# vlongle/pixie

Measured on AMD Instinct MI355X. Metric: voxels/s (128^3 U-Net fwd) + MPM particle-steps/s, higher is better.
Workload: dtype f32 (operands split fp16 hi+lo, 3 f16 MFMAs/product, fp32 accumulate); 1 GPU; 128^3x64 feature grid -> SegmentationUNet+RegressionUNet forward (+argmax/one-hot combine), 1 scene per GPU per step; grid=128, feature_channels=64, parallelism=scene-parallel x1, executor=c+hip_graph

## Files before the change

pixie_amd/csrc/conv16_body.h:

```cpp
#pragma once
#include <type_traits>

#include "conv16_device.h"

namespace pixie {

template <int KS, int MB, int NB, bool EX = false, bool SP = false, int SK = 0, bool PAIR = false>
__device__ __forceinline__ void conv3d_f16x3_body(const Conv16Args& A) {
    static_assert(!PAIR || (MB == 2 && !EX && !SP && SK == 0), "pair form: the plain f16x3 body with 64 c_out per quartet");
    static_assert(!SP || (KS == 3 && NB == 4 && !EX), "sub-pixel path: 3^3, two x parities x two voxel blocks per wave");
    static_assert(SK == 0 || (!EX && !SP), "folded skip (SK: 1 register-fed, 2 staged through LDS): f16x3, no sub-pixel form");
    extern __shared__ uint4 smem16[];
    constexpr int PAD = (KS == 3) ? 1 : 0;
    constexpr int NW = 4, NT = 64 * NW;
    const int bufsz = 4 * A.CS;

    const int tid = threadIdx.x;
    const int lane = tid & 63;
    const int quartet = PAIR ? __builtin_amdgcn_readfirstlane(tid >> 8) : 0;
    const int wave = PAIR ? (tid >> 6) & 3 : tid >> 6;
    const int qtid = PAIR ? tid & 255 : tid;
    const int kh = lane >> 5;
    const int l31 = lane & 31;

    int t = blockIdx.x;
    {
        const int per = (A.n_tiles + 7) >> 3;
        const int cand = (t & 7) * per + (t >> 3);
        if ((A.n_tiles & 7) == 0) t = cand;
    }
    int par = 0;
    if constexpr (SP) { par = t & 3; t >>= 2; }
    const int py = par & 1, pz = par >> 1;
    const int tx = t % A.tiles_x; t /= A.tiles_x;
    const int ty = t % A.tiles_y;
    const int tz = t / A.tiles_y;
    const int ox0 = tx * A.TX, oy0 = ty * A.TY, oz0 = tz * A.TZ;
    const int cout0 = (PAIR ? 2 * (int)blockIdx.y + quartet : (int)blockIdx.y) * (MB * 32);
    const int lx0 = SP ? ox0 - 1 : ox0 * A.stride - PAD;
    const int ly0 = SP ? oy0 - 1 + py : oy0 * A.stride - PAD;
    const int lz0 = SP ? oz0 - 1 + pz : oz0 * A.stride - PAD;
// ... 31 lines not shown
    }

    float bound = A.in_bound;
    if (A.amax0) {
        bound = __uint_as_float(*A.amax0);
        if (A.amax1) bound = fmaxf(bound, __uint_as_float(*A.amax1));
    }
    const int ex = EX ? 0 : scale_exponent(bound);
    const float sx = pow2i(ex);

    f32x16 acc[MB][NB];
#pragma unroll
    for (int mb = 0; mb < MB; ++mb)
#pragma unroll
        for (int nb = 0; nb < NB; ++nb)
#pragma unroll
            for (int r = 0; r < 16; ++r) acc[mb][nb][r] = 0.0f;

    const int KG = A.cin >> 3;
    const size_t tap_stride = (size_t)KG * A.coutp;
    const size_t plane = (size_t)(SP ? 64 : KS * KS * KS) * tap_stride;
    const uint4* wHi = A.w16 + kW16HeaderU4 + (size_t)kh * A.coutp + cout0 + l31 + (size_t)(par * 16) * tap_stride;
    const uint4* wLo = wHi + plane;
    const float* wF = A.wf + (size_t)kh * A.coutp + cout0 + l31;

    constexpr int TAPS = KS * KS * KS;
#include "conv16_stage.h"
#include "conv16_taps.h"

    float inv2 = 0.0f;
    {
        const int c_begin = A.partial ? (int)blockIdx.z * A.chunks_per_slice * 16 : 0;
        const int c_end = A.partial ? min(A.cin, c_begin + A.chunks_per_slice * 16) : A.cin;
        if constexpr (PAIR) {
            const int n_chunks = (c_end - c_begin) >> 4;
            const int half = (A.CS + 1) >> 1;
            const int s0 = quartet ? half : 0, s1 = quartet ? A.CS : half;
#pragma unroll 1
            for (int h = -1; h < 2 * n_chunks; ++h) {
                const int k = h >> 1;
                const bool stage = (h < 0 || ((h + quartet) & 1) == 0) && k + 1 < n_chunks;
                const bool multiply = h >= 0 && ((h + quartet) & 1) != 0;
                if (stage) stage_chunk(c_begin + 16 * (k + 1), smem16 + ((k + 1) & 1) * bufsz, qtid, NT, s0, s1);
                if (multiply) mfma_chunk(c_begin + 16 * k, smem16 + (k & 1) * bufsz);
                if (h & 1) __syncthreads();
            }
        } else {
            for (int c_base = c_begin; c_base < c_end; c_base += 16) {
                __syncthreads();
                stage_chunk(c_base, smem16, tid, NT, 0, A.CS);
                __syncthreads();
                mfma_chunk(c_base, smem16);
            }
        }
#include "conv16_skip.h"
    }

#include "conv16_epilogue.h"
}

template <int KS, int MB, int NB>
__global__ __launch_bounds__(256, 2) void conv3d_f16x3_kernel(Conv16Args A) {
    conv3d_f16x3_body<KS, MB, NB>(A);
}
template <int KS, int NB>
__global__ __launch_bounds__(512, 1) void conv3d_f16x3_pair_kernel(Conv16Args A) {
    conv3d_f16x3_body<KS, 2, NB, false, false, 0, true>(A);
}
template <int KS, int MB, int NB, bool STAGED>
__global__ __launch_bounds__(256, 2) void conv3d_f16x3_skip_kernel(Conv16Args A) {
    conv3d_f16x3_body<KS, MB, NB, false, false, STAGED ? 2 : 1>(A);
}
template <int KS, int MB, int NB>
__global__ __launch_bounds__(256, 2) void conv3d_exact_kernel(Conv16Args A) {
    conv3d_f16x3_body<KS, MB, NB, true>(A);
}
template <int MB>
__global__ __launch_bounds__(256, 2) void conv3d_f16x3_subpixel_kernel(Conv16Args A) {
    conv3d_f16x3_body<3, MB, 4, false, true>(A);
}
__global__ __launch_bounds__(256, 2) void conv3d_f16x3_c64_fullres_kernel(Conv16Args A) {
    conv3d_f16x3_body<3, 2, 4>(A);
}

}
```

pixie_amd/csrc/conv3d_f16x3.hip:

```cpp
#include <hip/hip_runtime.h>

#include <cstdlib>

#include "../../include/pixie_hip.h"
#include "common.h"
#include "conv_plan.h"
#include "conv_launch.h"
#include "conv16_device.h"
#include "conv16_body.h"
#include "conv_stat_kernels.h"
#include "conv_pack_kernels.h"

namespace pixie {

bool conv_exact_v1() { return getenv("PIXIE_CONV_EXACT_V1") != nullptr; }

ConvShape conv_shape_of(const pixie_conv_desc* d) {
    ConvShape s;
    s.c0 = d->c0; s.c1 = d->c1; s.c_out = d->c_out;
    s.in_d = d->in_d; s.in_h = d->in_h; s.in_w = d->in_w;
    s.ksize = d->ksize; s.stride = d->stride; s.upsample = d->upsample;
    s.out_d = d->out_d; s.out_h = d->out_h; s.out_w = d->out_w;
    s.skip_c0 = d->skip_c0; s.skip_c1 = d->skip_c1;
    s.w16 = d->d_w16 != nullptr; s.subpixel = d->w16_subpixel != 0; s.workspace = d->d_workspace != nullptr; s.skip = d->d_skip_w16 != nullptr;
    s.exact_v1 = conv_exact_v1();
    return s;
}

using ConvKernel = void (*)(Conv16Args);
static ConvKernel conv16_kernel(const ConvPlan& p, bool skip = false, int skip_c0 = 0) {
    if (p.path == CONV_F16X3_SUBPIXEL) return p.MB == 2 ? conv3d_f16x3_subpixel_kernel<2> : conv3d_f16x3_subpixel_kernel<1>;
    if (p.fullres) return conv3d_f16x3_c64_fullres_kernel;
#define PX_CONV16_PICK(KS_, MB_, NB_)                                                                \
    if (p.KS == KS_ && p.MB == MB_ && p.NB == NB_)                                                   \
        return p.path == CONV_EXACT_TILED ? conv3d_exact_kernel<KS_, MB_, NB_>                       \
                                          : (!skip ? conv3d_f16x3_kernel<KS_, MB_, NB_>                                \
                                                   : ((skip_c0 & 8) ? conv3d_f16x3_skip_kernel<KS_, MB_, NB_, true> : conv3d_f16x3_skip_kernel<KS_, MB_, NB_, false>));
    PX_CONV_VARIANTS(PX_CONV16_PICK)
#undef PX_CONV16_PICK
    return nullptr;
}

#ifdef PIXIE_DIAG
static int g_conv_keep_four_wave = 0;
#endif
static size_t conv_pair_lds(const ConvPlan& p, bool skip) {
#ifdef PIXIE_DIAG
    if (g_conv_keep_four_wave) return 0;
#endif
    return conv_pair_lds_bytes(p, skip);
}
static ConvKernel conv16_pair_kernel(const ConvPlan& p) {
#define PX_CONV16_PAIR(KS_, NB_) \
    if (p.KS == KS_ && p.NB == NB_) return conv3d_f16x3_pair_kernel<KS_, NB_>;
    PX_CONV16_PAIR(3, 4) PX_CONV16_PAIR(1, 4)
#undef PX_CONV16_PAIR
    return nullptr;
}

static int launch(ConvKernel kern, const ConvPlan& p, const Conv16Args& a, hipStream_t st, size_t pair_lds = 0) {
    PX_REQUIRE(kern != nullptr, "conv: no kernel variant for ksize=%d MB=%d NB=%d", p.KS, p.MB, p.NB);
    PX_CHECK_HIP(allow_max_dynamic_lds(reinterpret_cast<const void*>(kern)));
    if (pair_lds) hipLaunchKernelGGL(kern, dim3(p.grid_x, p.grid_y / 2, 1), dim3(512), pair_lds, st, a);
    else hipLaunchKernelGGL(kern, dim3(p.grid_x, p.grid_y, p.grid_z), dim3(256), p.lds_bytes, st, a);
    PX_CHECK_HIP(hipGetLastError());
    return 0;
}

static Conv16Args conv16_args(const pixie_conv_desc* d, const ConvPlan& p) {
    Conv16Args a{};
    a.in0 = d->d_in0; a.in1 = d->d_in1; a.c0 = d->c0; a.cin = d->c0 + d->c1;
    a.ID = d->in_d; a.IH = d->in_h; a.IW = d->in_w;
    a.LD = p.LD; a.LH = p.LH; a.LW = p.LW; a.ups = p.ups; a.stride = d->stride;
    a.OD = p.OD; a.OH = p.OH; a.OW = p.OW;
    a.pro_a = d->d_pro_a; a.pro_b = d->d_pro_b; a.gamma = d->d_gamma; a.beta = d->d_beta; a.act = d->act;
    a.bias = d->d_bias; a.cout = d->c_out; a.coutp = p.coutp;
    a.residual = d->d_residual; a.out = d->d_out;
    a.TX = p.TX; a.TY = p.TY; a.TZ = p.TZ; a.lTX = p.lTX; a.lTY = p.lTY;
    a.tiles_x = p.tiles_x; a.tiles_y = p.tiles_y; a.tiles_z = p.tiles_z; a.n_tiles = p.n_tiles;
    a.HX = p.HX; a.HY = p.HY; a.HZ = p.HZ; a.HYX = p.HYX; a.CS = p.CS; a.mHX = p.mHX; a.mHYX = p.mHYX;
    a.chunks_per_slice = p.chunks_per_slice; a.epi_lds = p.epi_lds;
    return a;
}

int conv3d_f16x3_forward(const pixie_conv_desc* d, const ConvPlan& p, hipStream_t st) {
    PX_REQUIRE(p.refusal != CONV_BAD_STRIDE, "f16x3 conv: stride must be 1, or 2 for a 3^3 kernel");
    PX_REQUIRE(p.refusal != CONV_BAD_CHANNELS, "f16x3 conv: c_in must be a multiple of 16 (got %d+%d)", d->c0, d->c1);
    PX_REQUIRE(d->d_in_amax0 != nullptr || d->in_bound > 0.0f, "f16x3 conv: needs d_in_amax0 or a positive in_bound");
    PX_REQUIRE(d->c1 == 0 || d->d_in_amax0 == nullptr || d->d_in_amax1 != nullptr, "f16x3 conv: second input needs its own amax slot");
    PX_REQUIRE(p.refusal != CONV_BAD_SUBPIXEL, "f16x3 conv: sub-pixel weights need upsample = 1, ksize = 3, stride = 1 and no folded skip");
    PX_REQUIRE((int64_t)d->in_d * d->in_h * d->in_w * 16 * (int64_t)sizeof(float) < (int64_t)1 << 32, "f16x3 conv: 16 channels of the input must span less than 4 GiB");
    Conv16Args a = conv16_args(d, p);
    a.w16 = reinterpret_cast<const uint4*>(d->d_w16);
    a.amax0 = d->d_in_amax0; a.amax1 = (d->c1 > 0) ? d->d_in_amax1 : nullptr; a.in_bound = d->in_bound;
    a.stats = d->d_out_stats; a.out_amax = d->d_out_amax;
    if (d->d_skip_w16) {
        PX_REQUIRE(p.skip_foldable, "f16x3 conv: this launch cannot fold a skip convolution (pixie_conv_skip_foldable)");
        PX_REQUIRE(d->d_skip_in0 && d->d_skip_amax0 && (d->skip_c1 == 0 || (d->d_skip_in1 && d->d_skip_amax1)), "f16x3 conv: folded skip needs its inputs and their amax slots");
        PX_REQUIRE((int64_t)d->in_d * d->in_h * d->in_w * 16 * (int64_t)sizeof(float) < (int64_t)1 << 32, "f16x3 conv: folded skip: 16 channels of the skip input must span less than 4 GiB");
        a.sk_in0 = d->d_skip_in0; a.sk_in1 = d->d_skip_in1; a.sk_c0 = d->skip_c0; a.sk_cin = d->skip_c0 + d->skip_c1;
        a.sk_w16 = reinterpret_cast<const uint4*>(d->d_skip_w16); a.sk_bias = d->d_skip_bias;
        a.sk_amax0 = d->d_skip_amax0; a.sk_amax1 = d->skip_c1 > 0 ? d->d_skip_amax1 : nullptr;
    }
    if (p.slices > 1) {
        a.partial = static_cast<float*>(d->d_workspace);
        a.stats = nullptr; a.out_amax = nullptr;
    }
    PX_REQUIRE(p.refusal != CONV_BAD_LDS, "f16x3 conv: tile needs %zu B of LDS", p.lds_bytes);
    PX_REQUIRE(p.f16x3(), "f16x3 conv: bad sizes");
    const size_t pair_lds = conv_pair_lds(p, a.sk_w16 != nullptr);
    if (int rc = launch(pair_lds ? conv16_pair_kernel(p) : conv16_kernel(p, a.sk_w16 != nullptr, a.sk_c0), p, a, st, pair_lds)) return rc;
    if (p.slices == 1) return 0;
    const long osp = (long)a.OD * a.OH * a.OW, n_elems = (long)a.cout * osp;
    if (d->d_out_stats) {
        const dim3 rgrid((unsigned)reduce_segments(osp), (unsigned)a.cout);
        double* rstats = reinterpret_cast<double*>(d->d_out_stats);
        PX_REQUIRE((reinterpret_cast<size_t>(rstats) & 7) == 0, "f16x3 conv: d_out_stats of a split-K launch must be 8-byte aligned");
        const bool vec = osp % 4 == 0 && ((reinterpret_cast<size_t>(a.partial) | reinterpret_cast<size_t>(a.residual) | reinterpret_cast<size_t>(a.out)) & 15) == 0;
        if (vec) hipLaunchKernelGGL(splitk_reduce_stats_kernel<true>, rgrid, dim3(256), 0, st, a.partial, p.slices, n_elems, osp, a.bias, a.residual,
                                    a.out, rstats, d->d_out_amax);
        else hipLaunchKernelGGL(splitk_reduce_stats_kernel<false>, rgrid, dim3(256), 0, st, a.partial, p.slices, n_elems, osp, a.bias, a.residual,
                                a.out, rstats, d->d_out_amax);
    } else {
        hipLaunchKernelGGL(splitk_reduce_kernel, dim3((unsigned)((n_elems + 255) / 256)), dim3(256), 0, st, a.partial, p.slices, n_elems, osp,
                           a.bias, a.residual, a.out);
    }
    PX_CHECK_HIP(hipGetLastError());
    return 0;
}

int conv3d_exact_forward(const pixie_conv_desc* d, const ConvPlan& p, hipStream_t st) {
    PX_REQUIRE(p.refusal != CONV_BAD_LDS, "exact conv: tile needs %zu B of LDS", p.lds_bytes);
    PX_REQUIRE(p.path == CONV_EXACT_TILED, "exact conv: bad sizes");
    Conv16Args a = conv16_args(d, p);
    a.wf = d->d_w;
    a.in_bound = 1.0f;
    return launch(conv16_kernel(p), p, a, st);
}

}

using namespace pixie;

static ConvPlan plan_of(const pixie_conv_desc* d) { return d ? conv_plan(conv_shape_of(d)) : ConvPlan{}; }
static StatParts stat_parts(const ConvPlan& p, const void* stats) { return StatParts{stats, p.stats.n, p.stats.cstride, p.stats.tstride, p.stats.f64}; }

extern "C" int64_t pixie_conv_stats_floats(const pixie_conv_desc* d) { return plan_of(d).stats_floats; }

extern "C" int64_t pixie_conv_workspace_bytes(const pixie_conv_desc* d) {
    if (!d) return 0;
    ConvShape s = conv_shape_of(d);
    s.workspace = true;
    return conv_plan(s).workspace_bytes;
}

#ifdef PIXIE_DIAG
extern "C" int pixie_conv_kernel_variant(const pixie_conv_desc* d, int* slices_out) {
    if (!d) {
        const int before = g_conv_keep_four_wave;
        if (slices_out && (*slices_out == 0 || *slices_out == 1)) g_conv_keep_four_wave = *slices_out;
        return before;
    }
    const ConvPlan p = plan_of(d);
    if (slices_out) *slices_out = p.f16x3() ? p.slices : 1;
    return conv_variant_number(p);
}

extern "C" int pixie_conv_tile_geometry(const pixie_conv_desc* d, int32_t out[10]) {
    const ConvPlan p = plan_of(d);
    if (!out && d) return (int)conv_pair_lds(p, d->d_skip_w16 != nullptr);
    return out && conv_tile_geometry(p, out) ? 0 : 1;
}

extern "C" int pixie_conv_stats_layout(const pixie_conv_desc* d, int64_t out[6]) {
    const ConvPlan p = plan_of(d);
    return out && conv_stats_layout(p, out) ? 0 : 1;
}
#endif

extern "C" int pixie_conv_skip_foldable(const pixie_conv_desc* d) { return plan_of(d).skip_foldable ? 1 : 0; }

extern "C" int pixie_stats_finalize(const float* d_stats, const pixie_conv_desc* d, double* d_sums, void* stream) {
    PX_REQUIRE(d_stats && d && d_sums, "pixie_stats_finalize: null argument");
    hipLaunchKernelGGL(stats_finalize_kernel, dim3((unsigned)d->c_out), dim3(256), 0, as_stream(stream), stat_parts(plan_of(d), d_stats), d_sums);
    PX_CHECK_HIP(hipGetLastError());
    return 0;
}

extern "C" int pixie_stats_norm_finalize(const float* d_stats0, const pixie_conv_desc* desc0, double* d_sums0, const float* d_stats1,
                                         const pixie_conv_desc* desc1, double* d_sums1, int c1, int64_t spatial, int mode, int groups,
                                         double eps, const float* d_weight, const float* d_bias, float* d_a, float* d_b, void* stream) {
    PX_REQUIRE(desc0 && d_sums0 && d_a && d_b && spatial > 0 && c1 >= 0, "pixie_stats_norm_finalize: bad arguments");
    PX_REQUIRE(c1 == 0 || d_sums1, "pixie_stats_norm_finalize: a second part needs d_sums1");
    PX_REQUIRE(!d_stats1 || desc1, "pixie_stats_norm_finalize: d_stats1 needs its descriptor");
    const int c0 = desc0->c_out, channels = c0 + c1;
    PX_REQUIRE(!d_stats1 || desc1->c_out == c1, "pixie_stats_norm_finalize: desc1 has %d output channels, c1 is %d", desc1 ? desc1->c_out : 0, c1);
    PX_REQUIRE(mode == 0 || (mode == 1 && groups > 0 && channels % groups == 0), "pixie_stats_norm_finalize: bad mode/groups");
    const StatParts none{nullptr, 0, 0, 0, 0};
    const StatParts p0 = d_stats0 ? stat_parts(plan_of(desc0), d_stats0) : none;
    const StatParts p1 = d_stats1 ? stat_parts(plan_of(desc1), d_stats1) : none;
    hipLaunchKernelGGL(stats_norm_finalize_kernel, dim3((unsigned)(mode == 0 ? channels : groups)), dim3(256), 0, as_stream(stream), p0, d_sums0, c0,
                       p1, d_sums1, channels, (double)spatial, mode, groups, eps, d_weight, d_bias, d_a, d_b);
    PX_CHECK_HIP(hipGetLastError());
    return 0;
}

extern "C" int64_t pixie_conv_packed16_bytes(int c_out, int c_in, int ksize) {
    if (c_out <= 0 || c_in <= 0 || c_in % 8 != 0 || (ksize != 1 && ksize != 3)) return 0;
    const int64_t taps = (int64_t)ksize * ksize * ksize;
    return ((int64_t)kW16HeaderU4 + 2 * taps * (c_in / 8) * pixie_conv_cout_padded(c_out)) * (int64_t)sizeof(uint4);
}

extern "C" int pixie_tensor_amax(const float* d_x, int64_t count, uint32_t* d_slot, void* stream) {
    PX_REQUIRE(d_x && d_slot && count > 0, "pixie_tensor_amax: bad arguments");
    const int blocks = (int)std::min<int64_t>(2048, (count + 1023) / 1024);
    hipLaunchKernelGGL(amax_kernel, dim3(blocks), dim3(256), 0, as_stream(stream), d_x, (long)count, d_slot);
    PX_CHECK_HIP(hipGetLastError());
    return 0;
}

extern "C" int pixie_conv_pack_weights_f16x2(const float* d_w, void* d_packed, int c_out, int c_in, int ksize, void* stream) {
    PX_REQUIRE(d_w && d_packed && c_out > 0 && c_in > 0 && c_in % 8 == 0 && (ksize == 1 || ksize == 3),
               "pixie_conv_pack_weights_f16x2: bad arguments (c_in must be a multiple of 8)");
    hipStream_t st = as_stream(stream);
    const int taps = ksize * ksize * ksize;
    const int coutp = pixie_conv_cout_padded(c_out);
    unsigned* slot = reinterpret_cast<unsigned*>(d_packed) + 15;
    PX_CHECK_HIP(hipMemsetAsync(d_packed, 0, kW16HeaderU4 * sizeof(uint4), st));
    if (pixie_tensor_amax(d_w, (int64_t)c_out * c_in * taps, slot, stream)) return 1;
    const long total = (long)taps * (c_in / 8) * coutp;
    hipLaunchKernelGGL(pack_weights_f16x2_kernel, dim3(cdiv(total, 256)), dim3(256), 0, st, d_w, reinterpret_cast<uint4*>(d_packed), c_out,
                       c_in, taps, coutp, slot);
    PX_CHECK_HIP(hipGetLastError());
    return 0;
}

extern "C" int64_t pixie_conv_subpixel_bytes(int c_out, int c_in) {
    if (c_out <= 0 || c_in <= 0 || c_in % 16 != 0) return 0;
    return ((int64_t)kW16HeaderU4 + 2 * 64 * (int64_t)(c_in / 8) * pixie_conv_cout_padded(c_out)) * (int64_t)sizeof(uint4);
}

extern "C" int pixie_conv_pack_weights_subpixel(const float* d_w, void* d_packed, int c_out, int c_in, void* stream) {
    PX_REQUIRE(d_w && d_packed && c_out > 0 && c_in > 0 && c_in % 16 == 0,
               "pixie_conv_pack_weights_subpixel: bad arguments (c_in must be a multiple of 16)");
    hipStream_t st = as_stream(stream);
    const int coutp = pixie_conv_cout_padded(c_out);
    unsigned* slot = reinterpret_cast<unsigned*>(d_packed) + 15;
    PX_CHECK_HIP(hipMemsetAsync(d_packed, 0, kW16HeaderU4 * sizeof(uint4), st));
// ... 10 lines not shown
```

pixie_amd/csrc/conv_plan.h:

```cpp
#pragma once
#include <algorithm>
#include <cstddef>
#include <cstdint>

#include "../../include/pixie_hip.h"

namespace pixie {

#define PX_CONV_VARIANTS(X) \
    X(3, 2, 4) X(3, 2, 2) X(3, 2, 1) X(3, 1, 4) X(3, 1, 2) X(3, 1, 1) X(1, 2, 4) X(1, 2, 2) X(1, 2, 1) X(1, 1, 4) X(1, 1, 2) X(1, 1, 1)

struct ConvShape {
    int c0 = 0, c1 = 0, c_out = 0, in_d = 0, in_h = 0, in_w = 0, ksize = 0, stride = 1, upsample = 0;
    int out_d = 0, out_h = 0, out_w = 0;
    int skip_c0 = 0, skip_c1 = 0;
    bool w16 = false;
    bool subpixel = false;
    bool workspace = false;
    bool skip = false;
    bool exact_v1 = false;
};

enum ConvPath { CONV_NONE = 0, CONV_F16X3, CONV_F16X3_SUBPIXEL, CONV_EXACT_TILED, CONV_FIRST_GEN };
enum ConvRefusal { CONV_OK = 0, CONV_BAD_SHAPE, CONV_BAD_STRIDE, CONV_BAD_CHANNELS, CONV_BAD_SUBPIXEL, CONV_BAD_LDS };
// ... 107 lines not shown
    if (p.slices > 1) p.chunks_per_slice = (chunks + p.slices - 1) / p.slices;
    p.lds_bytes = (size_t)4 * p.CS * 16;
    if (p.lds_bytes > 160 * 1024) return refuse(CONV_BAD_LDS);
    const size_t epi_bytes = ((size_t)4 * 32 * (p.NB * 32 + 4) + (size_t)4 * p.MB * 32 * 2) * sizeof(float);
    if (p.slices == 1 && epi_bytes <= 80 * 1024) { p.epi_lds = 1; p.lds_bytes = std::max(p.lds_bytes, epi_bytes); }
    p.grid_x = (unsigned)p.n_tiles; p.grid_y = (unsigned)((p.coutp + p.MB * 32 - 1) / (p.MB * 32)); p.grid_z = (unsigned)p.slices;
    if (!p.f16x3()) return p;
    const long osp = (long)p.OD * p.OH * p.OW;
    if (p.slices > 1) {
        const int n = reduce_segments(osp);
        p.stats = ConvStatLayout{n, n, 1, 1};
        p.stats_floats = (int64_t)s.c_out * n * 2 * (int64_t)(sizeof(double) / sizeof(float));
        p.workspace_bytes = (int64_t)p.slices * s.c_out * osp * (int64_t)sizeof(float);
    } else {
        p.stats = ConvStatLayout{p.n_tiles, 1, p.coutp, 0};
        p.stats_floats = (int64_t)p.n_tiles * p.coutp * 2;
    }
    p.fullres = !sub && p.slices == 1 && s.ksize == 3 && p.MB == 2 && p.NB == 4 && cin == 64 && s.c_out == 64 && s.stride == 1 && !s.upsample &&
                s.c1 == 0 && !s.skip && osp >= 128L * 128 * 128;
    const int scin = s.skip_c0 + s.skip_c1;
    p.skip_foldable = !sub && s.stride == 1 && !s.upsample && scin > 0 && scin % 16 == 0 && s.skip_c0 % 8 == 0 && p.slices == 1;
    return p;
}

inline size_t conv_pair_lds_bytes(const ConvPlan& p, bool skip) {
    if (p.path != CONV_F16X3 || p.fullres || skip || p.MB != 2 || p.NB != 4 || p.slices != 1 || p.coutp % 128 != 0) return 0;
    const size_t tiles = (size_t)2 * 4 * p.CS * 16;
    const size_t red = (size_t)2 * 4 * p.MB * 32 * 2 * sizeof(float);
    const size_t epi = p.epi_lds ? (size_t)8 * 32 * (p.NB * 32 + 4) * sizeof(float) + red : red;
    const size_t lds = std::max(tiles, epi);
    return lds <= 160 * 1024 ? lds : 0;
}

inline int conv_variant_number(const ConvPlan& p) {
    if (!p.f16x3()) return 0;
    if (p.path == CONV_F16X3_SUBPIXEL) return 8300 + p.MB * 10 + p.NB;
    if (p.fullres) return 9324;
    return p.KS * 100 + p.MB * 10 + p.NB;
}
inline bool conv_tile_geometry(const ConvPlan& p, int32_t out[10]) {
    if (!p.tiled()) return false;
    const int32_t v[10] = {p.TX, p.TY, p.TZ, p.tiles_x, p.tiles_y, p.tiles_z, p.epi_lds, p.slices, p.MB, p.NB};
    for (int i = 0; i < 10; ++i) out[i] = v[i];
    return true;
}
inline bool conv_stats_layout(const ConvPlan& p, int64_t out[6]) {
    if (!p.f16x3()) return false;
    out[0] = p.stats.n; out[1] = p.stats.cstride; out[2] = p.stats.tstride; out[3] = p.stats.f64; out[4] = p.stats.f64 ? kReduceSeg : 0;
    out[5] = p.coutp;
    return true;
}

}
```

pixie_amd/csrc/conv_stat_kernels.h:

```cpp
#pragma once
#include <hip/hip_runtime.h>

#include "conv_plan.h"

namespace pixie {

struct StatParts { const void* p; int n; long cstride, tstride; int f64; };

__device__ inline void block_channel_sums(const StatParts& P, int c, double* r, double& o1, double& o2) {
    double s1 = 0.0, s2 = 0.0;
    for (int t = threadIdx.x; t < P.n; t += 256) {
        const size_t k = ((size_t)c * P.cstride + (size_t)t * P.tstride) * 2;
        if (P.f64) { const double2 v = *reinterpret_cast<const double2*>(static_cast<const double*>(P.p) + k); s1 += v.x; s2 += v.y; }
        else { const float2 v = *reinterpret_cast<const float2*>(static_cast<const float*>(P.p) + k); s1 += v.x; s2 += v.y; }
    }
    for (int off = 32; off > 0; off >>= 1) { s1 += __shfl_down(s1, off, 64); s2 += __shfl_down(s2, off, 64); }
    if ((threadIdx.x & 63) == 0) { r[2 * (threadIdx.x >> 6)] = s1; r[2 * (threadIdx.x >> 6) + 1] = s2; }
    __syncthreads();
    o1 = r[0] + r[2] + r[4] + r[6]; o2 = r[1] + r[3] + r[5] + r[7];
    __syncthreads();
}

__global__ __launch_bounds__(256) void stats_finalize_kernel(StatParts P, double* __restrict__ sums) {
    const int c = blockIdx.x;
// ... 97 lines not shown
                for (int s = 1; s < slices; ++s) v += partial[(size_t)s * n_elems + i];
                if (bias) v += bv;
                if (residual) v += residual[i];
                out[i] = v;
                const double x = v;
                s1 += x; s2 += x * x; mx = fmaxf(mx, fabsf(v));
            }
        }
    }
    for (int off = 32; off > 0; off >>= 1) {
        s1 += __shfl_down(s1, off, 64);
        s2 += __shfl_down(s2, off, 64);
        mx = fmaxf(mx, __shfl_down(mx, off, 64));
    }
    __shared__ double r[8];
    __shared__ float rmx[4];
    const int lane = threadIdx.x & 63, wave = threadIdx.x >> 6;
    if (lane == 0) { r[2 * wave] = s1; r[2 * wave + 1] = s2; rmx[wave] = mx; }
    __syncthreads();
    if (threadIdx.x == 0) {
        double* dst = stats + ((size_t)c * gridDim.x + blockIdx.x) * 2;
        dst[0] = r[0] + r[2] + r[4] + r[6];
        dst[1] = r[1] + r[3] + r[5] + r[7];
        const unsigned m = __float_as_uint(fmaxf(fmaxf(rmx[0], rmx[1]), fmaxf(rmx[2], rmx[3])));
        if (out_amax && m > __hip_atomic_load(out_amax, __ATOMIC_RELAXED, __HIP_MEMORY_SCOPE_AGENT)) atomicMax(out_amax, m);
    }
}

__global__ __launch_bounds__(256) void amax_kernel(const float* __restrict__ x, long n, unsigned* __restrict__ slot) {
    float m = 0.0f;
    const long stride = (long)gridDim.x * 256 * 4;
    long i = ((long)blockIdx.x * 256 + threadIdx.x) * 4;
    if ((reinterpret_cast<size_t>(x) & 15) == 0) {
        for (; i + 3 < n; i += stride) {
            const float4 v = *reinterpret_cast<const float4*>(x + i);
            m = fmaxf(fmaxf(m, fabsf(v.x)), fmaxf(fabsf(v.y), fmaxf(fabsf(v.z), fabsf(v.w))));
        }
        for (long k = i; k < n && k < i + 4; ++k) m = fmaxf(m, fabsf(x[k]));
    } else {
        for (long k = (long)blockIdx.x * 256 + threadIdx.x; k < n; k += (long)gridDim.x * 256) m = fmaxf(m, fabsf(x[k]));
    }
    for (int off = 32; off > 0; off >>= 1) m = fmaxf(m, __shfl_down(m, off, 64));
    if ((threadIdx.x & 63) == 0 && m > 0.0f) atomicMax(slot, __float_as_uint(m));
}

}
```

pixie_amd/csrc/unet_exec.hip:

```cpp
#include <hip/hip_runtime.h>

#include <algorithm>
#include <cmath>
#include <cstdlib>
#include <cstring>
#include <map>
#include <memory>
#include <stdexcept>
#include <string>
#include <tuple>
#include <unordered_map>
#include <vector>

#include "../../include/pixie_hip.h"
#include "common.h"
#include "conv_launch.h"
#include "conv_plan.h"

namespace pixie {
int channel_stats_prezeroed(const float* d_x, int channels, int64_t spatial, double* d_sums, uint32_t* d_amax, hipStream_t st);
int norm_finalize_cat(const double* d_sums0, int c0, const double* d_sums1, int c1, int64_t spatial, int mode, int groups, double eps,
                      const float* d_weight, const float* d_bias, float* d_a, float* d_b, hipStream_t st);
namespace {

// ... 164 lines not shown
            if (off + bytes > peak) peak = off + bytes;
            return off;
        }
        fail("pixie_unet_forward: the workspace is too small (%lld bytes; ask pixie_unet_workspace_bytes for this grid size)", (long long)capacity);
    }
    void release(int64_t off) {
        auto u = used_.find(off);
        if (u == used_.end()) return;
        int64_t size = u->second;
        used_.erase(u);
        auto next = free_.lower_bound(off);
        if (next != free_.end() && off + size == next->first) { size += next->second; next = free_.erase(next); }
        if (next != free_.begin()) {
            auto prev = std::prev(next);
            if (prev->first + prev->second == off) { prev->second += size; return; }
        }
        free_[off] = size;
    }
    template <class T> T* ptr(int64_t off) const { return reinterpret_cast<T*>(base + off); }
};

struct Exec;
struct Tens {
    Exec* ex = nullptr;
    float* p = nullptr;
    int64_t off = -1;
    int c = 0, d = 0, h = 0, w = 0;
    int64_t sums_off = -1;
    bool has_sums = false;
    double* sums = nullptr;
    int64_t partials_off = -1;
    pixie_conv_desc pdesc;
    uint32_t* slot = nullptr;
    int64_t spatial() const { return (int64_t)d * h * w; }
    ~Tens();
};
using TP = std::shared_ptr<Tens>;

struct Packed { void* d = nullptr; uint64_t version = ~0ull; };
struct Sized { int64_t bytes; int slots; int64_t zsum_doubles; };
struct Bound { float wmax = 0, bmax = 0; uint64_t wver = ~0ull, bver = ~0ull; };

}
}

using namespace pixie;

struct pixie_unet {
    Cfg cfg;
    Plan plan;
    std::vector<Param> params;
    std::unordered_map<std::string, int> index;
    std::unordered_map<std::string, Packed> packed32, packed16;
    std::unordered_map<std::string, Bound> bounds;
    uint32_t* d_bound_slots = nullptr;
    std::vector<uint32_t> h_bound_slots;
    std::map<std::tuple<int, int, int, bool>, Sized> sized;
    bool fuse_stats = true, split_k = true, fold_skip = true, subpixel = true;
    bool split_stats = true;
    struct Replay { const float* feat; const float* proj0; float* out; void* ws; int d; uint64_t epoch; hipGraph_t graph; hipGraphExec_t exec; };
    bool use_graph = false;
    uint64_t epoch = 0;
    std::vector<Replay> replays;
    static constexpr size_t kMaxReplays = 4;
    void drop_replay(size_t i) {
        (void)hipGraphExecDestroy(replays[i].exec);
// ... 57 lines not shown
            const int cout = (int)p.shape[0], cin = (int)p.shape[1], k = (int)p.shape[2];
            const int64_t nb = subpixel ? (k == 3 ? pixie_conv_subpixel_bytes(cout, cin) : 0) : pixie_conv_packed16_bytes(cout, cin, k);
            if (nb <= 0) fail("pixie_unet: '%s' cannot take the f16x3 packing (c_in %d)", key.c_str(), cin);
            if (!e.d && hipMalloc(&e.d, (size_t)nb) != hipSuccess) fail("pixie_unet: hipMalloc of %lld bytes failed", (long long)nb);
            if (!p.d) fail("pixie_unet_forward: parameter '%s.weight' was never set", key.c_str());
            if (subpixel) ok(pixie_conv_pack_weights_subpixel(p.d, e.d, cout, cin, stream), "pixie_conv_pack_weights_subpixel");
            else ok(pixie_conv_pack_weights_f16x2(p.d, e.d, cout, cin, k, stream), "pixie_conv_pack_weights_f16x2");
            e.version = p.version;
        }
        return e.d;
    }
    const float* w32(const std::string& key) {
        const Param& p = net->param(key + ".weight");
        if (dry) return nullptr;
        Packed& e = net->packed32[key];
        if (e.version != p.version) {
            const int cout = (int)p.shape[0], cin = (int)p.shape[1], k = (int)p.shape[2];
            int64_t taps = 1;
            for (size_t i = 2; i < p.shape.size(); ++i) taps *= p.shape[i];
            const int64_t nb = taps * cin * pixie_conv_cout_padded(cout) * (int64_t)sizeof(float);
            if (!e.d && hipMalloc(&e.d, (size_t)nb) != hipSuccess) fail("pixie_unet: hipMalloc of %lld bytes failed", (long long)nb);
            if (!p.d) fail("pixie_unet_forward: parameter '%s.weight' was never set", key.c_str());
            ok(pixie_conv_pack_weights(p.d, static_cast<float*>(e.d), cout, cin, k, stream), "pixie_conv_pack_weights");
            e.version = p.version;
        }
        return static_cast<const float*>(e.d);
    }
    float norm_bound(const std::string& key, int64_t count) {
        if (dry) return 1.0f;
        const Bound& b = net->bounds[key];
        return (float)(std::sqrt((double)count) * (double)b.wmax + (double)b.bmax + 1e-30);
    }

    void stats(const TP& t) {
        if (t->has_sums || t->partials_off >= 0) return;
        t->has_sums = true;
        if (!dry && zsum_next + 2 * t->c > zsum_cap) fail("pixie_unet_forward: out of statistics space (internal sizing error)");
        t->sums = dry ? nullptr : zsums + zsum_next;
        zsum_next += 2 * t->c;
        t->slot = new_slot();
        if (!dry) ok(channel_stats_prezeroed(t->p, t->c, t->spatial(), t->sums, t->slot, as_stream(stream)), "pixie_channel_stats");
    }
    struct AB { std::shared_ptr<Scratch> mem; float* a; float* b; };
    AB norm_finalize(const std::vector<TP>& parts, int64_t spatial, int mode, int groups, const float* w, const float* b) {
        for (auto& t : parts) stats(t);
        const Tens* t0 = parts[0].get();
        const Tens* t1 = parts.size() > 1 ? parts[1].get() : nullptr;
        const int c0 = t0->c, c1 = t1 ? t1->c : 0, c = c0 + c1;
        AB r;
        const int cpad = (c + 63) / 64 * 64;
        r.mem = std::make_shared<Scratch>(this, (int64_t)(cpad + c) * sizeof(float));
        r.a = r.mem->as<float>();
        r.b = r.a + cpad;
        const bool p0 = t0->partials_off >= 0, p1 = t1 && t1->partials_off >= 0;
        if (p0 || p1) {
            pixie_conv_desc d0 = t0->pdesc;
            if (!p0) { std::memset(&d0, 0, sizeof d0); d0.c_out = c0; }
            if (!dry) ok(pixie_stats_norm_finalize(p0 ? arena.ptr<float>(t0->partials_off) : nullptr, &d0, t0->sums,
                                                   p1 ? arena.ptr<float>(t1->partials_off) : nullptr, p1 ? &t1->pdesc : nullptr, t1 ? t1->sums : nullptr,
                                                   c1, spatial, mode, groups, 1e-5, w, b, r.a, r.b, stream), "pixie_stats_norm_finalize");
            for (auto& t : parts)
                if (t->partials_off >= 0) { arena.release(t->partials_off); t->partials_off = -1; t->has_sums = true; }
        } else if (!t1) {
            if (!dry) ok(pixie_norm_finalize(t0->sums, c, spatial, mode, groups, 1e-5, w, b, r.a, r.b, stream), "pixie_norm_finalize");
        } else {
            if (!dry) ok(norm_finalize_cat(t0->sums, c0, t1->sums, c1, spatial, mode, groups, 1e-5, w, b, r.a, r.b, as_stream(stream)), "pixie_norm_finalize");
        }
        return r;
    }

    ConvPlan plan_conv(ConvShape& s, const std::vector<TP>& parts, int cout, int ksize, int stride, bool upsample) const {
        s.c0 = parts[0]->c; s.c1 = parts.size() > 1 ? parts[1]->c : 0; s.c_out = cout;
        s.in_d = parts[0]->d; s.in_h = parts[0]->h; s.in_w = parts[0]->w;
// ... 1 lines not shown
        s.w16 = net->cfg.precision == 0; s.workspace = net->split_k; s.exact_v1 = conv_exact_v1();
        ConvPlan p = conv_plan(s);
        if (p.refusal == CONV_BAD_CHANNELS) { s.w16 = s.subpixel = s.skip = false; p = conv_plan(s); }
        return p;
    }
    bool skip_foldable(const TP& x, int cout, int ksize, const std::vector<TP>& sp) const {
        ConvShape s;
        s.skip_c0 = sp[0]->c; s.skip_c1 = sp.size() > 1 ? sp[1]->c : 0;
        return plan_conv(s, {x}, cout, ksize, 1, false).skip_foldable;
    }

    struct ConvOpt {
        int stride = 1; bool upsample = false;
        const AB* pro = nullptr; std::string affine_store;
        int act = ACT_NONE; TP residual; float bound = 0.0f;
        int out_d = 0, out_h = 0, out_w = 0;
        float* out_ptr = nullptr;
        const std::vector<TP>* skip_parts = nullptr; std::string skip_key;
    };
    TP conv(const std::vector<TP>& parts, const std::string& wkey, int cout, int ksize, const ConvOpt& o) {
        const TP& x0 = parts[0];
        const Tens* x1 = parts.size() > 1 ? parts[1].get() : nullptr;
        ConvShape s;
        s.out_d = o.out_d; s.out_h = o.out_h; s.out_w = o.out_w;
        s.subpixel = net->subpixel && o.upsample && ksize == 3 && o.stride == 1;
        if (o.skip_parts) { s.skip = true; s.skip_c0 = (*o.skip_parts)[0]->c; s.skip_c1 = o.skip_parts->size() > 1 ? (*o.skip_parts)[1]->c : 0; }
        const ConvPlan plan = plan_conv(s, parts, cout, ksize, o.stride, o.upsample);
        const int od = plan.OD, oh = plan.OH, ow = plan.OW;
        pixie_conv_desc desc;
        std::memset(&desc, 0, sizeof desc);
        if (o.out_d) { desc.out_d = od; desc.out_h = oh; desc.out_w = ow; }
        const bool f16 = s.w16;
        const bool raw = !o.pro && o.affine_store.empty();
        if (f16 && raw) for (auto& t : parts) stats(t);

        TP out = o.out_ptr ? external(o.out_ptr, cout, od, oh, ow) : make(cout, od, oh, ow);
        desc.d_in0 = x0->p; desc.c0 = x0->c;
        desc.d_in1 = x1 ? x1->p : nullptr; desc.c1 = x1 ? x1->c : 0;
        desc.in_d = x0->d; desc.in_h = x0->h; desc.in_w = x0->w;
        desc.upsample = o.upsample ? 1 : 0;
        desc.stride = o.stride;
        desc.ksize = ksize;
        if (o.pro) { desc.d_pro_a = o.pro->a; desc.d_pro_b = o.pro->b; }
        if (!o.affine_store.empty()) { desc.d_gamma = P(o.affine_store + ".weight"); desc.d_beta = P(o.affine_store + ".bias"); }
        desc.act = o.act;
        desc.d_bias = P(wkey + ".bias");
        desc.c_out = cout;
        desc.d_residual = o.residual ? o.residual->p : nullptr;
        desc.d_out = out->p;
        if (!f16) {
            desc.d_w = w32(wkey);
            if (!dry) ok(pixie_conv3d_forward(&desc, stream), "pixie_conv3d_forward");
            return out;
        }
        desc.d_w16 = w16(wkey, s.subpixel);
        desc.w16_subpixel = s.subpixel ? 1 : 0;
        if (o.skip_parts) {
            const std::vector<TP>& sp = *o.skip_parts;
            desc.d_skip_in0 = sp[0]->p; desc.skip_c0 = sp[0]->c;
            desc.d_skip_in1 = sp.size() > 1 ? sp[1]->p : nullptr; desc.skip_c1 = sp.size() > 1 ? sp[1]->c : 0;
            desc.d_skip_w16 = w16(o.skip_key);
            desc.d_skip_bias = P(o.skip_key + ".bias");
            desc.d_skip_amax0 = sp[0]->slot; desc.d_skip_amax1 = sp.size() > 1 ? sp[1]->slot : nullptr;
        }
        if (raw) {
            desc.d_in_amax0 = parts[0]->slot;
            desc.d_in_amax1 = x1 ? parts[1]->slot : nullptr;
// ... 5 lines not shown
        bool have_stats = false;
        if (net->fuse_stats) {
            uint32_t* slot = new_slot();
            const int64_t nfl = plan.stats_floats;
            if (nfl > 0 && (!workspace || net->split_stats)) {
                out->partials_off = arena.alloc(nfl * (int64_t)sizeof(float));
                desc.d_out_stats = arena.ptr<float>(out->partials_off);
                desc.d_out_amax = slot;
                have_stats = true;
                out->slot = slot;
            }
        }
        if (!dry) ok(pixie_conv3d_forward(&desc, stream), "pixie_conv3d_forward");
        if (have_stats) {
            out->sums_off = arena.alloc((int64_t)cout * 2 * sizeof(double));
            out->sums = arena.ptr<double>(out->sums_off);
            out->pdesc = desc;
        }
        return out;
    }

    TP res(const Blk& b, const std::vector<TP>& parts) {
        const std::string& p = b.prefix;
        const int64_t spatial = parts[0]->spatial();
        AB pro = norm_finalize(parts, spatial, 0, 1, nullptr, nullptr);
        ConvOpt o1; o1.pro = &pro; o1.affine_store = p + ".in_layers.0"; o1.act = ACT_LEAKY; o1.bound = norm_bound(p + ".in_layers.0", spatial);
        TP h = conv(parts, p + ".in_layers.2", b.cout, 3, o1);
        AB pro2 = norm_finalize({h}, spatial, 0, 1, nullptr, nullptr);
        TP skip = parts[0];
        ConvOpt o2; o2.pro = &pro2; o2.affine_store = p + ".out_layers.0"; o2.act = ACT_LEAKY; o2.bound = norm_bound(p + ".out_layers.0", spatial);
        if (b.cin != b.cout) {
            if (net->fold_skip && skip_foldable(h, b.cout, 3, parts)) {
                skip.reset();
                for (auto& t : parts) stats(t);
                o2.skip_parts = &parts; o2.skip_key = p + ".skip_connection";
            } else {
                skip = conv(parts, p + ".skip_connection", b.cout, 1, ConvOpt{});
            }
        }
        o2.residual = skip;
        return conv({h}, p + ".out_layers.3", b.cout, 3, o2);
    }
    TP attn(const Blk& b, const TP& x) {
        const std::string& p = b.prefix;
        const int c = x->c;
        const int64_t spatial = x->spatial();
        AB pro = norm_finalize({x}, spatial, 1, 32, P(p + ".norm.weight"), P(p + ".norm.bias"));
        ConvOpt o; o.pro = &pro; o.bound = norm_bound(p + ".norm", spatial * (c / 32));
        TP qkv = conv({x}, p + ".qkv", 3 * c, 1, o);
        TP att = make(c, x->d, x->h, x->w);
        if (!dry) ok(pixie_attention_forward(qkv->p, att->p, c, (int)spatial, stream), "pixie_attention_forward");
        qkv.reset();
        ConvOpt o2; o2.residual = x;
        return conv({att}, p + ".proj_out", c, 1, o2);
    }
    TP block(const Blk& b, const std::vector<TP>& parts, const Tens* up_to) {
        if (b.kind == RES) return res(b, parts);
        const TP& x = parts[0];
        if (b.kind == ATTN) return attn(b, x);
        if (b.kind == DOWN) { ConvOpt o; o.stride = 2; return conv({x}, b.prefix + ".op", b.cout, 3, o); }
        if (b.kind == UP) {
            ConvOpt o; o.upsample = true;
            if (up_to) { o.out_d = up_to->d; o.out_h = up_to->h; o.out_w = up_to->w; }
            return conv({x}, b.prefix + ".conv", b.cout, 3, o);
        }
        fail("pixie_unet: unexpected block kind");
    }
// ... 279 lines not shown
```

Baseline: 27.38 million voxels/s.

## Add register-fed 1x1 conv path, lighter amax-only input scaling, faster amax reduction

Adds a register-fed main loop for 1x1x1 f16x3 convolutions. It loads input voxels directly with buffer loads, applies the prologue affine and activation in registers, and issues MFMAs without staging through LDS or block barriers. Raw conv inputs now compute only an abs-max scale slot instead of full per-channel statistics, which saves a reduction pass. The amax kernel gets a 4x unrolled vector loop, fewer blocks, and a block-level reduction that issues one guarded atomic per block. The trade-off is more registers and more kernel variants, and fewer amax blocks may lower parallelism on small tensors.

After: 27.36 million voxels/s. No clear change (-0.1%).

```diff
diff --git a/pixie_amd/csrc/conv16_body.h b/pixie_amd/csrc/conv16_body.h
--- a/pixie_amd/csrc/conv16_body.h
+++ b/pixie_amd/csrc/conv16_body.h
@@ -5,8 +5,9 @@
 
 namespace pixie {
 
-template <int KS, int MB, int NB, bool EX = false, bool SP = false, int SK = 0, bool PAIR = false>
+template <int KS, int MB, int NB, bool EX = false, bool SP = false, int SK = 0, bool PAIR = false, bool RF = false>
 __device__ __forceinline__ void conv3d_f16x3_body(const Conv16Args& A) {
+    static_assert(!RF || (KS == 1 && !EX && !SP && SK == 0), "register-fed main loop: the plain f16x3 body, one tap, no folded skip");
     static_assert(!PAIR || (MB == 2 && !EX && !SP && SK == 0), "pair form: the plain f16x3 body with 64 c_out per quartet");
     static_assert(!SP || (KS == 3 && NB == 4 && !EX), "sub-pixel path: 3^3, two x parities x two voxel blocks per wave");
     static_assert(SK == 0 || (!EX && !SP), "folded skip (SK: 1 register-fed, 2 staged through LDS): f16x3, no sub-pixel form");
@@ -104,7 +105,9 @@
     {
         const int c_begin = A.partial ? (int)blockIdx.z * A.chunks_per_slice * 16 : 0;
         const int c_end = A.partial ? min(A.cin, c_begin + A.chunks_per_slice * 16) : A.cin;
-        if constexpr (PAIR) {
+        if constexpr (RF) {
+#include "conv16_single_tap.h"
+        } else if constexpr (PAIR) {
             const int n_chunks = (c_end - c_begin) >> 4;
             const int half = (A.CS + 1) >> 1;
             const int s0 = quartet ? half : 0, s1 = quartet ? A.CS : half;
@@ -139,6 +142,14 @@
 __global__ __launch_bounds__(512, 1) void conv3d_f16x3_pair_kernel(Conv16Args A) {
     conv3d_f16x3_body<KS, 2, NB, false, false, 0, true>(A);
 }
+template <int MB, int NB>
+__global__ __launch_bounds__(256, 2) void conv3d_f16x3_single_tap_kernel(Conv16Args A) {
+    conv3d_f16x3_body<1, MB, NB, false, false, 0, false, true>(A);
+}
+template <int NB>
+__global__ __launch_bounds__(512, 1) void conv3d_f16x3_single_tap_pair_kernel(Conv16Args A) {
+    conv3d_f16x3_body<1, 2, NB, false, false, 0, true, true>(A);
+}
 template <int KS, int MB, int NB, bool STAGED>
 __global__ __launch_bounds__(256, 2) void conv3d_f16x3_skip_kernel(Conv16Args A) {
     conv3d_f16x3_body<KS, MB, NB, false, false, STAGED ? 2 : 1>(A);
diff --git a/pixie_amd/csrc/conv16_single_tap.h b/pixie_amd/csrc/conv16_single_tap.h
--- /dev/null
+++ b/pixie_amd/csrc/conv16_single_tap.h
@@ -0,0 +1,87 @@
+        {
+            const unsigned chb = 4u * (unsigned)ISP;
+            unsigned off[NB];
+#pragma unroll
+            for (int nb = 0; nb < NB; ++nb) {
+                const int j = (wave * NB + nb) * 32 + l31;
+                const int x = j & (A.TX - 1), y = (j >> A.lTX) & (A.TY - 1), z = j >> (A.lTX + A.lTY);
+                off[nb] = (valid[nb] ? 4u * (unsigned)(((oz0 + z) * A.IH + (oy0 + y)) * A.IW + ox0 + x) : 0u) + 8u * (unsigned)kh * chb;
+            }
+            auto rf_chunks = [&](auto has_pro, auto act_c) {
+#pragma unroll 1
+                for (int c_base = c_begin; c_base < c_end; c_base += 16) {
+                    f16x8 ah[MB], al[MB];
+                    const uint4* wh = wHi + (size_t)(c_base >> 3) * A.coutp;
+                    const uint4* wl = wLo + (size_t)(c_base >> 3) * A.coutp;
+#pragma unroll
+                    for (int mb = 0; mb < MB; ++mb) {
+                        al[mb] = __builtin_bit_cast(f16x8, wl[mb * 32]);
+                        ah[mb] = __builtin_bit_cast(f16x8, wh[mb * 32]);
+                    }
+                    float pa[8], pb[8];
+                    if constexpr (decltype(has_pro)::value) {
+#pragma unroll
+                        for (int q = 0; q < 8; ++q) {
+                            pa[q] = A.pro_a[c_base + 8 * kh + q];
+                            pb[q] = A.pro_b[c_base + 8 * kh + q];
+                        }
+                    }
+                    const float* base = (c_base < A.c0) ? (A.in0 + (size_t)c_base * ISP) : (A.in1 + (size_t)(c_base - A.c0) * ISP);
+                    const __amdgpu_buffer_rsrc_t rsrc = __builtin_amdgcn_make_buffer_rsrc(const_cast<float*>(base), 0, -1, 0x00020000);
+                    float v[NB][8];
+#pragma unroll
+                    for (int q = 0; q < 8; ++q)
+#pragma unroll
+                        for (int nb = 0; nb < NB; ++nb)
+                            v[nb][q] = __uint_as_float(__builtin_amdgcn_raw_buffer_load_b32(rsrc, (int)off[nb], (int)((unsigned)q * chb), 0));
+                    __builtin_amdgcn_sched_barrier(0);
+                    const float gm = 1.0f, bt = 0.0f;
+                    f16x8 bh[NB], bl[NB];
+#pragma unroll
+                    for (int nb = 0; nb < NB; ++nb) {
+                        f16x8 vh, vl;
+#pragma unroll
+                        for (int q = 0; q < 8; ++q) {
+                            float t = v[nb][q];
+                            if constexpr (decltype(has_pro)::value) t = t * pa[q] + pb[q];
+                            t = t * gm + bt;
+                            const float sc = act16_staged(t, decltype(act_c)::value) * sx;
+                            const _Float16 h = (_Float16)sc;
+                            vh[q] = h;
+                            vl[q] = (_Float16)(sc - (float)h);
+                        }
+                        uint4 w[2] = {__builtin_bit_cast(uint4, vh), __builtin_bit_cast(uint4, vl)};
+#pragma unroll
+                        for (int q = 0; q < 2; ++q) {
+                            w[q].x = valid[nb] ? w[q].x : 0u; w[q].y = valid[nb] ? w[q].y : 0u;
+                            w[q].z = valid[nb] ? w[q].z : 0u; w[q].w = valid[nb] ? w[q].w : 0u;
+                        }
+                        bh[nb] = __builtin_bit_cast(f16x8, w[0]);
+                        bl[nb] = __builtin_bit_cast(f16x8, w[1]);
+                    }
+#pragma unroll
+                    for (int mb = 0; mb < MB; ++mb)
+#pragma unroll
+                        for (int nb = 0; nb < NB; ++nb)
+                            acc[mb][nb] = __builtin_amdgcn_mfma_f32_32x32x16_f16(al[mb], bh[nb], acc[mb][nb], 0, 0, 0);
+#pragma unroll
+                    for (int mb = 0; mb < MB; ++mb)
+#pragma unroll
+                        for (int nb = 0; nb < NB; ++nb)
+                            acc[mb][nb] = __builtin_amdgcn_mfma_f32_32x32x16_f16(ah[mb], bl[nb], acc[mb][nb], 0, 0, 0);
+#pragma unroll
+                    for (int mb = 0; mb < MB; ++mb)
+#pragma unroll
+                        for (int nb = 0; nb < NB; ++nb)
+                            acc[mb][nb] = __builtin_amdgcn_mfma_f32_32x32x16_f16(ah[mb], bh[nb], acc[mb][nb], 0, 0, 0);
+                    __builtin_amdgcn_sched_barrier(0);
+                }
+            };
+            using T = std::true_type; using F = std::false_type;
+            if (A.pro_a) {
+                if (A.act == 2) rf_chunks(T{}, std::integral_constant<int, 2>{});
+                else rf_chunks(T{}, std::integral_constant<int, 0>{});
+            } else {
+                rf_chunks(F{}, std::integral_constant<int, 0>{});
+            }
+        }
diff --git a/pixie_amd/csrc/conv3d_f16x3.hip b/pixie_amd/csrc/conv3d_f16x3.hip
--- a/pixie_amd/csrc/conv3d_f16x3.hip
+++ b/pixie_amd/csrc/conv3d_f16x3.hip
@@ -43,12 +43,27 @@
 
 #ifdef PIXIE_DIAG
 static int g_conv_keep_four_wave = 0;
+static int g_conv_single_tap_launches = 0;
 #endif
 static size_t conv_pair_lds(const ConvPlan& p, bool skip) {
 #ifdef PIXIE_DIAG
-    if (g_conv_keep_four_wave) return 0;
+    if (g_conv_keep_four_wave & 1) return 0;
 #endif
     return conv_pair_lds_bytes(p, skip);
+}
+static bool conv_single_tap(const pixie_conv_desc* d, const ConvPlan& p) {
+#ifdef PIXIE_DIAG
+    if (g_conv_keep_four_wave & 2) return false;
+#endif
+    return conv_single_tap_registers(p, d->c0, d->d_pro_a != nullptr, d->act, d->d_gamma != nullptr, d->d_skip_w16 != nullptr);
+}
+static ConvKernel conv16_single_tap_kernel(const ConvPlan& p, bool pair) {
+    if (pair) return p.NB == 4 ? conv3d_f16x3_single_tap_pair_kernel<4> : nullptr;
+#define PX_CONV16_SINGLE_TAP(MB_, NB_) \
+    if (p.MB == MB_ && p.NB == NB_) return conv3d_f16x3_single_tap_kernel<MB_, NB_>;
+    PX_CONV_SINGLE_TAP_VARIANTS(PX_CONV16_SINGLE_TAP)
+#undef PX_CONV16_SINGLE_TAP
+    return nullptr;
 }
 static ConvKernel conv16_pair_kernel(const ConvPlan& p) {
 #define PX_CONV16_PAIR(KS_, NB_) \
@@ -109,7 +124,13 @@
     PX_REQUIRE(p.refusal != CONV_BAD_LDS, "f16x3 conv: tile needs %zu B of LDS", p.lds_bytes);
     PX_REQUIRE(p.f16x3(), "f16x3 conv: bad sizes");
     const size_t pair_lds = conv_pair_lds(p, a.sk_w16 != nullptr);
-    if (int rc = launch(pair_lds ? conv16_pair_kernel(p) : conv16_kernel(p, a.sk_w16 != nullptr, a.sk_c0), p, a, st, pair_lds)) return rc;
+    const bool single_tap = conv_single_tap(d, p);
+    const ConvKernel kern = single_tap ? conv16_single_tap_kernel(p, pair_lds != 0)
+                                       : (pair_lds ? conv16_pair_kernel(p) : conv16_kernel(p, a.sk_w16 != nullptr, a.sk_c0));
+#ifdef PIXIE_DIAG
+    g_conv_single_tap_launches += single_tap ? 1 : 0;
+#endif
+    if (int rc = launch(kern, p, a, st, pair_lds)) return rc;
     if (p.slices == 1) return 0;
     const long osp = (long)a.OD * a.OH * a.OW, n_elems = (long)a.cout * osp;
     if (d->d_out_stats) {
@@ -157,8 +178,9 @@
 #ifdef PIXIE_DIAG
 extern "C" int pixie_conv_kernel_variant(const pixie_conv_desc* d, int* slices_out) {
     if (!d) {
+        if (slices_out && *slices_out == 4) return g_conv_single_tap_launches;
         const int before = g_conv_keep_four_wave;
-        if (slices_out && (*slices_out == 0 || *slices_out == 1)) g_conv_keep_four_wave = *slices_out;
+        if (slices_out && *slices_out >= 0 && *slices_out <= 3) g_conv_keep_four_wave = *slices_out;
         return before;
     }
     const ConvPlan p = plan_of(d);
@@ -213,7 +235,7 @@
 
 extern "C" int pixie_tensor_amax(const float* d_x, int64_t count, uint32_t* d_slot, void* stream) {
     PX_REQUIRE(d_x && d_slot && count > 0, "pixie_tensor_amax: bad arguments");
-    const int blocks = (int)std::min<int64_t>(2048, (count + 1023) / 1024);
+    const int blocks = (int)std::min<int64_t>(2048, (count + 4095) / 4096);
     hipLaunchKernelGGL(amax_kernel, dim3(blocks), dim3(256), 0, as_stream(stream), d_x, (long)count, d_slot);
     PX_CHECK_HIP(hipGetLastError());
     return 0;
diff --git a/pixie_amd/csrc/conv_plan.h b/pixie_amd/csrc/conv_plan.h
--- a/pixie_amd/csrc/conv_plan.h
+++ b/pixie_amd/csrc/conv_plan.h
@@ -163,6 +163,18 @@
     return lds <= 160 * 1024 ? lds : 0;
 }
 
+#define PX_CONV_SINGLE_TAP_VARIANTS(X) X(2, 4) X(2, 2) X(2, 1) X(1, 4) X(1, 1)
+inline bool conv_single_tap_registers(const ConvPlan& p, int c0, bool pro, int act, bool spatial_affine, bool skip) {
+    if (p.path != CONV_F16X3 || p.KS != 1 || p.ups != 0) return false;
+    if (spatial_affine || skip || c0 % 16 != 0) return false;
+    if (pro ? (act != 0 && act != 2) : act != 0) return false;
+#define PX_CONV_SINGLE_TAP_HAS(MB_, NB_) \
+    if (p.MB == MB_ && p.NB == NB_) return true;
+    PX_CONV_SINGLE_TAP_VARIANTS(PX_CONV_SINGLE_TAP_HAS)
+#undef PX_CONV_SINGLE_TAP_HAS
+    return false;
+}
+
 inline int conv_variant_number(const ConvPlan& p) {
     if (!p.f16x3()) return 0;
     if (p.path == CONV_F16X3_SUBPIXEL) return 8300 + p.MB * 10 + p.NB;
diff --git a/pixie_amd/csrc/conv_stat_kernels.h b/pixie_amd/csrc/conv_stat_kernels.h
--- a/pixie_amd/csrc/conv_stat_kernels.h
+++ b/pixie_amd/csrc/conv_stat_kernels.h
@@ -153,6 +153,13 @@
     const long stride = (long)gridDim.x * 256 * 4;
     long i = ((long)blockIdx.x * 256 + threadIdx.x) * 4;
     if ((reinterpret_cast<size_t>(x) & 15) == 0) {
+        for (; i + 3 * stride + 3 < n; i += 4 * stride) {
+            float4 v[4];
+#pragma unroll
+            for (int u = 0; u < 4; ++u) v[u] = *reinterpret_cast<const float4*>(x + i + u * stride);
+#pragma unroll
+            for (int u = 0; u < 4; ++u) m = fmaxf(fmaxf(m, fabsf(v[u].x)), fmaxf(fabsf(v[u].y), fmaxf(fabsf(v[u].z), fabsf(v[u].w))));
+        }
         for (; i + 3 < n; i += stride) {
             const float4 v = *reinterpret_cast<const float4*>(x + i);
             m = fmaxf(fmaxf(m, fabsf(v.x)), fmaxf(fabsf(v.y), fmaxf(fabsf(v.z), fabsf(v.w))));
@@ -162,7 +169,13 @@
         for (long k = (long)blockIdx.x * 256 + threadIdx.x; k < n; k += (long)gridDim.x * 256) m = fmaxf(m, fabsf(x[k]));
     }
     for (int off = 32; off > 0; off >>= 1) m = fmaxf(m, __shfl_down(m, off, 64));
-    if ((threadIdx.x & 63) == 0 && m > 0.0f) atomicMax(slot, __float_as_uint(m));
+    __shared__ float wm[4];
+    if ((threadIdx.x & 63) == 0) wm[threadIdx.x >> 6] = m;
+    __syncthreads();
+    if (threadIdx.x == 0) {
+        const unsigned bits = __float_as_uint(fmaxf(fmaxf(wm[0], wm[1]), fmaxf(wm[2], wm[3])));
+        if (bits > __hip_atomic_load(slot, __ATOMIC_RELAXED, __HIP_MEMORY_SCOPE_AGENT)) atomicMax(slot, bits);
+    }
 }
 
 }
diff --git a/pixie_amd/csrc/unet_exec.hip b/pixie_amd/csrc/unet_exec.hip
--- a/pixie_amd/csrc/unet_exec.hip
+++ b/pixie_amd/csrc/unet_exec.hip
@@ -220,6 +220,7 @@
     int64_t partials_off = -1;
     pixie_conv_desc pdesc;
     uint32_t* slot = nullptr;
+    bool has_amax = false;
     int64_t spatial() const { return (int64_t)d * h * w; }
     ~Tens();
 };
@@ -343,13 +344,20 @@
         return (float)(std::sqrt((double)count) * (double)b.wmax + (double)b.bmax + 1e-30);
     }
 
+    void input_scale(const TP& t) {
+        if (t->has_sums || t->partials_off >= 0 || t->has_amax) return;
+        t->has_amax = true;
+        t->slot = new_slot();
+        if (!dry) ok(pixie_tensor_amax(t->p, (int64_t)t->c * t->spatial(), t->slot, stream), "pixie_tensor_amax");
+    }
     void stats(const TP& t) {
         if (t->has_sums || t->partials_off >= 0) return;
         t->has_sums = true;
         if (!dry && zsum_next + 2 * t->c > zsum_cap) fail("pixie_unet_forward: out of statistics space (internal sizing error)");
         t->sums = dry ? nullptr : zsums + zsum_next;
         zsum_next += 2 * t->c;
-        t->slot = new_slot();
+        if (!t->has_amax) t->slot = new_slot();
+        t->has_amax = true;
         if (!dry) ok(channel_stats_prezeroed(t->p, t->c, t->spatial(), t->sums, t->slot, as_stream(stream)), "pixie_channel_stats");
     }
     struct AB { std::shared_ptr<Scratch> mem; float* a; float* b; };
@@ -417,7 +425,7 @@
         if (o.out_d) { desc.out_d = od; desc.out_h = oh; desc.out_w = ow; }
         const bool f16 = s.w16;
         const bool raw = !o.pro && o.affine_store.empty();
-        if (f16 && raw) for (auto& t : parts) stats(t);
+        if (f16 && raw) for (auto& t : parts) input_scale(t);
 
         TP out = o.out_ptr ? external(o.out_ptr, cout, od, oh, ow) : make(cout, od, oh, ow);
         desc.d_in0 = x0->p; desc.c0 = x0->c;
@@ -489,7 +497,7 @@
         if (b.cin != b.cout) {
             if (net->fold_skip && skip_foldable(h, b.cout, 3, parts)) {
                 skip.reset();
-                for (auto& t : parts) stats(t);
+                for (auto& t : parts) input_scale(t);
                 o2.skip_parts = &parts; o2.skip_key = p + ".skip_connection";
             } else {
                 skip = conv(parts, p + ".skip_connection", b.cout, 1, ConvOpt{});
```
